# OpenVQE/OpenVQE

Hardware: AMD Instinct MI355X
Metric: vqe_energy_evals_per_sec (higher is better)
Workload: dtype f64; 1 GPU; H2O/STO-3G UCCSD energy evaluation (the metric's config): 14 qubits, 140 generators = 1000 Pauli rotations, JW Hamiltonian 1086 terms / 162 x-groups; batch_per_gpu=65536, parallelism=batch-replicas x1

## Files before the change

### openvqe_amd/csrc/abi_eval.inc

```

int ovqe_set_hamiltonian(ovqe_handle h, int64_t T, const uint64_t *x, const uint64_t *z, const double *coeff,
                         double constant) try {
    OVQE_ENTER(h);
    if (!h || T < 0 || (T && (!x || !z || !coeff))) return OVQE_ERR_INVALID;
    int rc = install_hamdev(h, h->ham, T, x, z, coeff, constant);
    if (rc) return rc;
    free_sector(h->scr);
    h->scr_failed_version = -1;
    h->user_x.assign(x, x + T);
    h->user_z.assign(z, z + T);
    h->user_c.assign(coeff, coeff + T);
    h->user_const = constant;
    h->exp_lbits = -1;
    h->sp_tried = false;
    return install_conjugated_hamiltonian(h);
} OVQE_CATCH(h)

struct FrameHamGuard {
    ovqe_handle h;
    bool on;
    explicit FrameHamGuard(ovqe_handle hh) : h(hh), on(hh && hh->frame_open && hh->ham_conj.set) {
        if (on) std::swap(h->ham, h->ham_conj);
    }
    ~FrameHamGuard() {
// ... 202 lines not shown
            }
            use_cc = C.valid;
        }
        if (use_cc && real && h->opt_sector && h->sec.valid && !h->sec.h_tables && h->sec.K == h->cc.K) {
            double2 res;
            bool ok = false;
            rc = run_sector_state(h, theta + b * (int64_t)K, (double *)h->cc.d_psic.p, &ok);
            if (rc) return rc;
            if (ok) {
                rc = run_expectation_compact(h, h->ham_real, &res, &ok, true);
                if (rc) return rc;
            }
            if (ok) {
                energies[b] = res.x + h->ham.constant;
                continue;
            }
            sector_orphaned(h);
        }
        lap("before the dense run");
        rc = run_program_streaming(h, theta + b * (int64_t)K, real);
        if (rc) return rc;
        lap("dense run");
        double2 res;
        bool tiled = false;
        if (use_cc) {
            rc = run_expectation_compact(h, h->ham_real, &res, &tiled);
            if (rc) return rc;
            if (!tiled) {
                h->cc.valid = false;
                h->cc.disabled = true;
            }
        }
        if (!tiled) rc = run_expectation_tiled(h, real ? h->ham_real : h->ham, &res, &tiled, real);
        if (rc) return rc;
        if (real && !tiled) return fail(h, OVQE_ERR_INVALID, "internal: real-amplitude path without a tile cover");
        if (!tiled)
            rc = run_bilinear(h, h->state, h->state, h->ham.groups, (const HGroup *)h->ham.d_groups.p,
                              (const HTerm *)h->ham.d_terms.p, &res, true);
        if (rc) return rc;
        lap("dense <H>");
        energies[b] = res.x + h->ham.constant;
    }
    if (!timed) {
        h->last_batch_ms = 0.f;
        return OVQE_OK;
    }
    HIPC(h, hipEventRecord(h->ev1, h->stream));
    HIPC(h, hipStreamSynchronize(h->stream));
    HIPC(h, hipEventElapsedTime(&h->last_batch_ms, h->ev0, h->ev1));
    return OVQE_OK;
} OVQE_CATCH(h)

int ovqe_energy_batch_device(ovqe_handle h, int64_t B, const void *theta_dev, int32_t K, void *energies_dev) try {
    OVQE_ENTER(h);
    if (!h || B < 0 || (B && (!theta_dev || !energies_dev))) return OVQE_ERR_INVALID;
    FrameHamGuard frame_guard(h);
    if (!h->prog_set) return fail(h, OVQE_ERR_STATE, "no program set (ovqe_set_program / ovqe_set_gate_program)");
    if (K != h->K || K <= 0) return fail(h, OVQE_ERR_INVALID, "K does not match the program's parameter count");
    if (!h->ham.set) return fail(h, OVQE_ERR_STATE, "no Hamiltonian set (ovqe_set_hamiltonian)");
    if (B == 0) return OVQE_OK;
    int rc;
    if (h->opt_force_path == 0 || h->opt_force_path == 3) {
        if (!h->sp_tried) {
            rc = build_sparse_program(h);
            if (rc) return rc;
        }
        if (h->sp_valid) {
            bool done = false;
            rc = run_sparse(h, B, (const double *)theta_dev, (double *)energies_dev, true, &done);
            if (rc || done) return rc;
        } else {
            h->sp_forms |= SPF_DECLINED;
        }
        if (h->opt_force_path == 3) return fail(h, OVQE_ERR_STATE, "program has no compact form (sparse path forced)");
    }
    if (h->n_global == 0 && h->n_local <= 16 && h->opt_force_path != 2)
        return run_small(h, B, (const double *)theta_dev, (double *)energies_dev, true);
    if (h->opt_sector_batch && h->opt_real_stream && h->prog_real_ok && h->n_global == 0 && tile_ok(h, true) && h->ham.groups.size() >= 3) {
        rc = sector_prepare(h, true);
        if (rc) return rc;
        if (sector_batch_ready(h)) {
            bool ok = false;
            rc = run_sector_energy_batch(h, B, (const double *)theta_dev, true, (double *)energies_dev, &ok);
            if (rc) return rc;
            if (ok) return OVQE_OK;
        }
    }
    std::vector<double> th((size_t)B * K), en((size_t)B);
    HIPC(h, hipMemcpyAsync(th.data(), theta_dev, th.size() * sizeof(double), hipMemcpyDeviceToHost, h->stream));
    HIPC(h, hipStreamSynchronize(h->stream));
    rc = ovqe_energy_batch(h, B, th.data(), K, en.data());
    if (rc) return rc;
    HIPC(h, hipMemcpyAsync(energies_dev, en.data(), en.size() * sizeof(double), hipMemcpyHostToDevice, h->stream));
    HIPC(h, hipStreamSynchronize(h->stream));
    return OVQE_OK;
} OVQE_CATCH(h)

int ovqe_energy(ovqe_handle h, const double *theta, int32_t K, double *energy) try {
    OVQE_ENTER(h);
    return ovqe_energy_batch(h, 1, theta, K, energy);
} OVQE_CATCH(h)

static int list_support(ovqe_handle h, uint64_t *support, bool *listed, uint64_t capacity) {
    *support = 0;
    *listed = false;
    if (h->opt_screen_sparse <= 0 || h->n_global != 0 || h->namps < 4096) return OVQE_OK;
    const uint64_t per_block = 256ull * NZ_PER_THREAD;
    const unsigned nbk = (unsigned)((h->namps + per_block - 1) / per_block);
    int rc = ensure(h, h->d_nz_cnt, (size_t)nbk * sizeof(uint32_t));
    if (!rc) rc = ensure(h, h->d_nz_start, (size_t)nbk * sizeof(uint64_t));
    if (rc) return rc;
    hipLaunchKernelGGL(k_nz_count, dim3(nbk), dim3(256), 0, h->stream, (const amp_t *)h->state, h->namps, (uint32_t *)h->d_nz_cnt.p);
    std::vector<uint32_t> cnt(nbk);
    hipError_t e = hipMemcpyAsync(cnt.data(), h->d_nz_cnt.p, (size_t)nbk * sizeof(uint32_t), hipMemcpyDeviceToHost, h->stream);
    if (e == hipSuccess) e = hipStreamSynchronize(h->stream);
    if (e != hipSuccess) return fail(h, OVQE_ERR_HIP, std::string("support list: ") + hipGetErrorString(e));
    std::vector<uint64_t> start(nbk);
    uint64_t total = 0;
    for (unsigned b = 0; b < nbk; ++b) {
        start[b] = total;
        total += cnt[b];
    }
    *support = total;
    if (total == 0 || total * (uint64_t)h->opt_screen_sparse > h->namps) return OVQE_OK;
    rc = upload(h, h->d_nz_start, start.data(), (size_t)nbk * sizeof(uint64_t));
    if (!rc) rc = ensure(h, h->d_nz_idx, std::max(total, capacity) * sizeof(uint64_t));
    if (!rc) rc = ensure(h, h->d_nz_val, total * sizeof(amp_t));
    if (rc) return rc;
    hipLaunchKernelGGL(k_nz_fill, dim3(nbk), dim3(256), 0, h->stream, (const amp_t *)h->state, h->namps,
                       (const uint64_t *)h->d_nz_start.p, (uint64_t *)h->d_nz_idx.p, (amp_t *)h->d_nz_val.p);
// ... 139 lines not shown
```

### openvqe_amd/csrc/gates_host.inc

```

void push_gate(ovqe_handle h, int opcode, int b0, int b1) {
    SmallOp op = {};
    if (opcode == OVQE_GATE_CNOT) {
        op.x = 1ull << b1;
        op.kind = OP_CNOT;
        op.first = b0;
        op.count = b1;
        op.pivot = b1;
    } else {
        op.x = 1ull << b0;
        op.kind = opcode == OVQE_GATE_X ? OP_X : OP_H;
        op.pivot = b0;
    }
    h->ops.push_back(op);
}

void push_literal_gate(ovqe_handle h, int opcode, int b0, int b1, double ascale, double aconst, int32_t pidx) {
    const uint64_t bit = 1ull << b0;
    switch (opcode) {
    case OVQE_GATE_RX: push_rotation(h, bit, 0, 0.5 * ascale, 0.5 * aconst, pidx); break;
    case OVQE_GATE_RY: push_rotation(h, bit, bit, 0.5 * ascale, 0.5 * aconst, pidx); break;
    case OVQE_GATE_RZ: push_rotation(h, 0, bit, 0.5 * ascale, 0.5 * aconst, pidx); break;
    default: push_gate(h, opcode, b0, b1);
    }
// ... 357 lines not shown
        if (poll) poll_arm(h->h_io + (size_t)B * h->K, B);
        h->cur_theta = h->d_io;
        h->cur_energies = h->d_io + (size_t)B * h->K;
    } else if (!on_device) {
        rc = ensure(h, h->d_theta, (size_t)B * std::max(1, h->K) * sizeof(double));
        if (rc) return rc;
        rc = ensure(h, h->d_energies, (size_t)B * sizeof(double));
        if (rc) return rc;
        if (h->K > 0)
            HIPC(h, hipMemcpyAsync(h->d_theta.p, theta, (size_t)B * h->K * sizeof(double), hipMemcpyHostToDevice,
                                   h->stream));
        h->cur_theta = (const double *)h->d_theta.p;
        h->cur_energies = (double *)h->d_energies.p;
    }
    SmallArgs A;
    A.n = n;
    A.K = h->K;
    A.nsegs = (int)h->segs.size();
    A.ngroups = h->exp_ngroups;
    A.nchunks = h->exp_nchunks;
    A.nflat = h->exp_nflat;
    A.cs_capacity = h->cs_capacity;
    A.B = B;
    A.constant = h->ham.constant;
    A.hf = h->hf;
    const size_t smem = small_lds(real, lds_state, n, h->cs_capacity).bytes;
    if (!zero_copy) HIPC(h, hipEventRecord(h->ev0, h->stream));
    if (real) {
        if (!lds_state) rc = launch_small<true, false, 1024, 10>(h, A, grid, smem);
        else if (nt == 1024) rc = launch_small<true, true, 1024, 10>(h, A, grid, smem);
        else if (nt == 256) rc = launch_small<true, true, 256, 8>(h, A, grid, smem);
        else rc = launch_small<true, true, 64, 6>(h, A, grid, smem);
    } else {
        if (!lds_state) rc = launch_small<false, false, 1024, 10>(h, A, grid, smem);
        else if (nt == 1024) rc = launch_small<false, true, 1024, 10>(h, A, grid, smem);
        else if (nt == 256) rc = launch_small<false, true, 256, 8>(h, A, grid, smem);
        else rc = launch_small<false, true, 64, 6>(h, A, grid, smem);
    }
    if (rc) return rc;
    h->fused_launch[0] = (real ? 1 : 0) | (lds_state ? 2 : 0) | ((nt == 1024 ? 2 : (nt == 256 ? 1 : 0)) << 2) | (zero_copy ? 16 : 0) |
                         (poll ? 32 : 0) | (on_device ? 64 : 0);
    h->fused_launch[1] = grid;
    h->fused_launch[2] = A.nsegs;
    h->fused_launch[3] = A.nchunks;
    h->fused_launch[4] = A.ngroups;
    h->fused_launch[5] = A.nflat;
    if (zero_copy) {
        if (!poll || !poll_mapped_slots(h->h_io + (size_t)B * h->K, B)) HIPC(h, hipStreamSynchronize(h->stream));
        std::memcpy(energies, h->h_io + (size_t)B * h->K, (size_t)B * sizeof(double));
        h->last_batch_ms = 0.f;
        return OVQE_OK;
    }
    HIPC(h, hipEventRecord(h->ev1, h->stream));
    if (!on_device)
        HIPC(h, hipMemcpyAsync(energies, h->cur_energies, (size_t)B * sizeof(double), hipMemcpyDeviceToHost, h->stream));
    HIPC(h, hipStreamSynchronize(h->stream));
    HIPC(h, hipEventElapsedTime(&h->last_batch_ms, h->ev0, h->ev1));
    return OVQE_OK;
}
```

### openvqe_amd/csrc/ovqe_sv.hip

```cpp
#include "../../include/ovqe_sv.h"

#include <hip/hip_runtime.h>

#include <algorithm>
#include <type_traits>
#include <atomic>
#include <cmath>
#include <cstdio>
#include <complex>
#include <cstring>
#include <map>
#include <memory>
#include <numeric>
#include <string>
#include <thread>
#include <chrono>
#include <vector>

#include "sv_kernels.hpp"
#include "sv_small.hpp"
#include "sv_sparse.hpp"
#include "sparse_pack.hpp"
#include "sv_tile.hpp"
#include "sv_sector.hpp"
// ... 332 lines not shown
    int opt_sparse_renumber = 1;
    int opt_sparse_rows = 1;
    int opt_sparse_wg = 1;
    int opt_sparse_shared = 1;
    int opt_sparse_grad = 1;
    DevBuf d_egroups, d_eterms, d_echunks, d_eflat;
    int exp_lbits = -1, exp_real = -1, exp_ngroups = 0, exp_nchunks = 0, exp_nflat = 0;
    int exp_ham_version = -1;
    hipEvent_t ev0 = nullptr, ev1 = nullptr;
    hipStream_t stream2 = nullptr;
    hipEvent_t ev_fork = nullptr, ev_join = nullptr;
    int opt_real_state = 0;
    CompactCover cc;
    int opt_compact = 1;
    int prog_version = 0;
    SectorEngine sec;
    SectorEngine scr;
    int scr_failed_version = -1;
    bool probe_independent = false;
    int opt_sector = 1;
    int opt_sector_bits = 0;
    int opt_sector_max_gb = 128;
    int opt_sector_threads = 0;
    int opt_sector_min_qubits = 18;
    int opt_sector_h = 1;
    int opt_sector_h_bits = 0;
    int opt_sector_dict = 1;
    int opt_lanczos_keep_gb = 160;
    int opt_sector_tile_cap = 6500;
    int opt_sector_sparsity = 4;
    int opt_sector_profile = 0;
    int opt_sector_debug = 0;
    int opt_sector_stream_arrange = 1;
    int opt_sector_stream_waves = 0;
    int opt_sector_sweep = 3;
    int opt_sector_sweep_dbg = 0;
    int opt_sector_h_pack = 1;
    int opt_sector_h_dbg = 0;
    int opt_sector_adjoint = 3;
    int opt_screen_sector = 1;
    int opt_screen_sector_min = 1024;
    bool prog_from_gates = false;
    int opt_expect_dense = 1;
    DevBuf d_tile_cnt;
    int opt_tile_flat = 2;
    int opt_sector_eager_rots = 2048;
    int opt_sector_regular = 1;
    int opt_sector_reg_threads = 256;
    int opt_sector_reg_adjoint = 1;
    int opt_sector_reg_pairs = 1;
    int opt_sector_reg_runs = 1;
    int opt_sector_batch = 1;
    float last_batch_ms = 0.f;
    const double *cur_theta = nullptr;
    double *cur_energies = nullptr;
    int opt_force_path = 0;
    int opt_small_max = 14;
    int opt_small_batch_max = 16;
    int opt_index_streams = 1;
    int opt_table_fusion = 1;
    int64_t last_passes = 0;
    int64_t last_pass_bytes = 0;
    int64_t last_fci_rounds = 0;
    int fault_inject = 0;
    int opt_real_mode = 1;
    int opt_tile_bits = -1;
    double2 init_amp = make_double2(1.0, 0.0);
    int opt_clifford_frame = 1;
    int opt_tile_low = 4;
    TilePlan tp;
    TilePlan tp_real;
    bool tp_real_built = false;
    bool prog_real_ok = false;
    int opt_apply_min_tiles = 256;
    int opt_real_stream = 1;
    HamDev ham_real;
    TilePlan tp_adhoc;
    TilePlan tp_adjoint;
    int opt_adjoint_tile_bits = -1;
    int num_cus = 0;
    std::vector<CrossSum *> xsums;
    std::vector<PoolPlan *> xpools;
    RdmDev *rdm = nullptr;
    int opt_rdm_workspace_mb = 1024;
    MetricDev *metric = nullptr;
    int opt_metric_workspace_mb = 0;
    MeasureDev *measure = nullptr;
    SubspaceDev *subspace = nullptr;
    int opt_subspace_workspace_mb = 0;
    HessianDev *hessian = nullptr;
};

namespace {

int rebuild_small_program(ovqe_handle h);
int build_tile_program(ovqe_handle h);
bool mapped_io(ovqe_handle h, int64_t B);

int fail(ovqe_handle h, int code, const std::string &msg) {
    if (h) h->err = msg; else g_create_error = msg;
    return code;
}

int translate_exception(ovqe_handle h) noexcept {
    int code = OVQE_ERR_INVALID;
    try {
        try {
            throw;
        } catch (const std::bad_alloc &) {
            code = OVQE_ERR_ALLOC;
            fail(h, code, "host allocation failed (std::bad_alloc)");
        } catch (const std::exception &e) {
            fail(h, code, std::string("C++ exception stopped at the ABI: ") + e.what());
        } catch (...) {
            fail(h, code, "unknown C++ exception stopped at the ABI");
        }
    } catch (...) {
    }
    return code;
}
#define OVQE_CATCH(h) catch (...) { return translate_exception(h); }

#define OVQE_ENTER(h)                        \
    do {                                     \
        if (h) {                             \
            (void)hipSetDevice((h)->device); \
            (h)->nz_super_prev = (h)->nz_super; \
            (h)->nz_super = false;           \
        }                                    \
    } while (0)

#define HIPC(h, call)                                                                                   \
    do {                                                                                                \
        hipError_t e_ = (call);                                                                         \
        if (e_ != hipSuccess)                                                                           \
            return fail(h, OVQE_ERR_HIP, std::string(#call) + ": " + hipGetErrorString(e_));            \
    } while (0)

constexpr size_t LDS_WG_MAX = 160 * 1024;
constexpr size_t LDS_WG_BUDGET = 150 * 1024;
constexpr size_t LDS_TWO_PER_CU = 80 * 1024;
constexpr size_t SEC_LDS_MAX = 156 * 1024;

template <auto Kernel>
int lds_opt_in(ovqe_handle h, size_t bytes) {
    static std::atomic<bool> done[64];
    std::atomic<bool> &d = done[h->device & 63];
    if (!d.load(std::memory_order_acquire)) {
        HIPC(h, hipFuncSetAttribute(reinterpret_cast<const void *>(Kernel), hipFuncAttributeMaxDynamicSharedMemorySize, (int)bytes));
        d.store(true, std::memory_order_release);
    }
    return OVQE_OK;
}
template <auto K0, auto K1, auto... Ks>
int lds_opt_in(ovqe_handle h, size_t bytes) {
    const int rc = lds_opt_in<K0>(h, bytes);
    return rc ? rc : lds_opt_in<K1, Ks...>(h, bytes);
}

void free_hamdev(HamDev &H) {
    for (DevBuf *b : {&H.d_groups, &H.d_terms, &H.d_tchunks, &H.d_tgroups, &H.d_tterms, &H.d_tflats, &H.d_titems, &H.d_rest, &H.d_achunks,
                      &H.d_agroups, &H.d_aterms, &H.d_dzin, &H.d_doff, &H.d_dterms})
        if (b->p) {
            (void)hipFree(b->p);
            *b = DevBuf{};
        }
}

void free_cross_sum(CrossSum *X) {
    if (!X) return;
    free_hamdev(X->local);
    for (DevBuf *b : {&X->local_cover.d_achunks, &X->local_cover.d_agroups, &X->local_cover.d_aterms, &X->local_cover.d_groups, &X->local_cover.d_terms})
        if (b->p) (void)hipFree(b->p);
    for (int f = 0; f < 2; ++f)
        for (CrossCoverDev &C : X->partners[f])
            for (DevBuf *b : {&C.d_achunks, &C.d_agroups, &C.d_aterms, &C.d_groups, &C.d_terms})
                if (b->p) (void)hipFree(b->p);
    if (X->d_part.p) (void)hipFree(X->d_part.p);
    delete X;
}

void free_pool_plan(PoolPlan *P) {
    if (!P) return;
    for (int f = 0; f < 2; ++f)
        for (PoolCoverDev &D : P->covers[f])
            for (DevBuf *b : {&D.d_chunks, &D.d_entries, &D.d_terms})
                if (b->p) (void)hipFree(b->p);
    for (DevBuf *b : {&P->d_part, &P->d_out})
        if (b->p) (void)hipFree(b->p);
    delete P;
}

void release_block(void *p, size_t cap) {
    if (!p) return;
    if (DevBlockCache::current && DevBlockCache::current->blocks.size() < 512) DevBlockCache::current->blocks.push_back(DevBuf{p, cap});
    else (void)hipFree(p);
}

constexpr uint64_t OVQE_POLL_SENTINEL = 0x7ff8dead0badf00dull;
inline bool poll_mapped_slot(volatile uint64_t *slot) {
    const auto t0 = std::chrono::steady_clock::now();
    for (uint32_t spins = 0; *slot == OVQE_POLL_SENTINEL; ++spins) {
        __builtin_ia32_pause();
        if ((spins & 1023u) == 1023u && std::chrono::steady_clock::now() - t0 > std::chrono::milliseconds(5)) return false;
    }
    std::atomic_thread_fence(std::memory_order_acquire);
    return true;
}

inline void poll_arm(double *slots, int64_t B) {
    for (int64_t b = 0; b < B; ++b) std::memcpy(slots + b, &OVQE_POLL_SENTINEL, sizeof(uint64_t));
}
inline bool poll_mapped_slots(double *slots, int64_t B) {
    for (int64_t b = 0; b < B; ++b)
        if (!poll_mapped_slot(reinterpret_cast<volatile uint64_t *>(slots + b))) return false;
    return true;
}

int ensure(ovqe_handle h, DevBuf &b, size_t bytes) {
    if (b.cap >= bytes && b.p) return OVQE_OK;
    release_block(b.p, b.cap);
    b.p = nullptr;
    b.cap = 0;
    size_t want = std::max<size_t>(bytes, 256);
    if (DevBlockCache::current) {
        if (want < ((size_t)8 << 20)) {
            size_t base = 256;
            while (base * 2 <= want) base *= 2;
            const size_t step = base / 4;
            want = base + ((want - base + step - 1) / step) * step;
        }
        size_t cap = 0;
        if (void *p = DevBlockCache::current->take(want, &cap)) {
            b.p = p;
            b.cap = cap;
            return OVQE_OK;
        }
    }
    hipError_t e = hipMalloc(&b.p, want);
    if (e != hipSuccess && DevBlockCache::current && !DevBlockCache::current->blocks.empty()) {
        (void)hipGetLastError();
        DevBlockCache::current->flush();
        e = hipMalloc(&b.p, want);
    }
    if (e != hipSuccess) return fail(h, OVQE_ERR_ALLOC, std::string("hipMalloc: ") + hipGetErrorString(e));
    b.cap = want;
    return OVQE_OK;
}

int ensure_scratch(ovqe_handle h, int k) {
    if (h->scratch[k]) return OVQE_OK;
    hipError_t e = hipMalloc((void **)&h->scratch[k], h->namps * sizeof(amp_t));
    if (e != hipSuccess) return fail(h, OVQE_ERR_ALLOC, std::string("hipMalloc scratch: ") + hipGetErrorString(e));
    return OVQE_OK;
}

inline uint64_t local_mask(ovqe_handle h) { return h->namps - 1ull; }
inline int reduce_blocks(uint64_t namps) {
    return (int)std::min<uint64_t>(2048, std::max<uint64_t>(1, (namps + 255) / 256));
}

inline int enqueue_reduce(ovqe_handle h, const void *partials, int64_t count, int slot = 0) {
    hipLaunchKernelGGL(k_reduce, dim3(1), dim3(256), 0, h->stream, (const double2 *)partials, count, (double2 *)h->d_result.p, slot);
    HIPC(h, hipGetLastError());
    return OVQE_OK;
}
inline int fetch_result(ovqe_handle h, double2 *out, int nslots = 1) {
    HIPC(h, hipMemcpyAsync(h->h_result, h->d_result.p, (size_t)nslots * sizeof(double2), hipMemcpyDeviceToHost, h->stream));
    HIPC(h, hipStreamSynchronize(h->stream));
    std::copy(h->h_result, h->h_result + nslots, out);
    return OVQE_OK;
}
inline int reduce_to_host(ovqe_handle h, const void *partials, int64_t count, double2 *out) {
// ... 1 lines not shown
    return fetch_result(h, out);
}
inline int reduce_to_host(ovqe_handle h, const void *partials, int64_t count, double *re) {
    double2 sum = make_double2(0.0, 0.0);
    const int rc = reduce_to_host(h, partials, count, &sum);
    *re = sum.x;
    return rc;
}

int build_groups(ovqe_handle h, int64_t T, const uint64_t *x, const uint64_t *z, const double *cr, const double *ci,
                 bool allow_global_x, std::vector<HGroup> &groups, std::vector<HTerm> &terms,
                 std::vector<uint64_t> *xs_out = nullptr, std::vector<int64_t> *perm_out = nullptr) {
    const uint64_t lmask = local_mask(h);
    const int ntot = h->n_local + h->n_global;
    const uint64_t allmask = ntot >= 64 ? ~0ull : ((1ull << ntot) - 1ull);
    if (h->fault_inject == 1) {
        h->fault_inject = 0;
        throw std::bad_alloc();
    }
    std::vector<int64_t> order(T);
    std::iota(order.begin(), order.end(), 0);
    std::stable_sort(order.begin(), order.end(), [&](int64_t a, int64_t b) { return x[a] < x[b]; });
    groups.clear();
    terms.clear();
    terms.reserve(T);
    for (int64_t oi = 0; oi < T; ++oi) {
        const int64_t t = order[oi];
        if ((x[t] | z[t]) & ~allmask) return fail(h, OVQE_ERR_INVALID, "Pauli mask has bits beyond the register");
        if (!allow_global_x && (x[t] & ~lmask))
            return fail(h, OVQE_ERR_INVALID,
                        "x mask touches global (rank) bits: exchange shards first (openvqe_amd/distributed.py)");
        HTerm ht;
        ht.z = z[t];
        fold_iny(cr[t], ci ? ci[t] : 0.0, __builtin_popcountll(x[t] & z[t]), ht.cr, ht.ci);
        if (groups.empty() || x[order[oi - 1]] != x[t]) {
            HGroup g;
            g.x = x[t] & lmask;
            g.jbase = (h->base ^ x[t]) & ~lmask;
            g.t0 = (int32_t)terms.size();
            g.t1 = g.t0;
            g.tiny = 0.0;
            groups.push_back(g);
        }
        terms.push_back(ht);
        groups.back().t1 = (int32_t)terms.size();
        groups.back().tiny += 64.0 * 2.220446049250313e-16 * (std::fabs(ht.cr) + std::fabs(ht.ci));
        if (xs_out) xs_out->push_back(x[t] & lmask);
    }
    if (perm_out) *perm_out = order;
    return OVQE_OK;
}

int upload(ovqe_handle h, DevBuf &b, const void *src, size_t bytes) {
    int rc = ensure(h, b, bytes);
    if (rc) return rc;
    if (bytes) HIPC(h, hipMemcpyAsync(b.p, src, bytes, hipMemcpyHostToDevice, h->stream));
    HIPC(h, hipStreamSynchronize(h->stream));
    return OVQE_OK;
}

int launch_rot_run(ovqe_handle h, uint64_t x, const RotParam *d_rp, int nrot) {
    if (nrot <= 0) return OVQE_OK;
    const int nl = h->n_local;
    if (x == 0) {
        const uint64_t n = h->namps;
#define OVQE_LAUNCH_D(NT, U, NTL)                                                                                \
    hipLaunchKernelGGL((k_rot_diag_v<NT, U, NTL>), dim3((unsigned)((n + (uint64_t)NT * U - 1) / ((uint64_t)NT * U))), \
                       dim3(NT), 0, h->stream, h->state, n, h->base, d_rp, nrot);
        if (nl >= 32) {
            OVQE_LAUNCH_D(64, 4, true)
        } else if (nl >= 21 && nl < 25) {
            OVQE_LAUNCH_D(256, 1, false)
        } else if (nl >= 14) {
            OVQE_LAUNCH_D(64, 1, true)
        } else if (n >= 256u * 4u) {
            hipLaunchKernelGGL(k_rot_diag<4>, dim3((unsigned)((n + 1023) / 1024)), dim3(256), 0, h->stream, h->state,
                               n, h->base, d_rp, nrot);
        } else {
            hipLaunchKernelGGL(k_rot_diag<1>, dim3((unsigned)((n + 255) / 256)), dim3(256), 0, h->stream, h->state,
                               n, h->base, d_rp, nrot);
        }
#undef OVQE_LAUNCH_D
    } else {
        const uint64_t np = h->namps >> 1;
        const int pivot = 63 - __builtin_clzll(x);
#define OVQE_LAUNCH_V(NT, U, NTL)                                                                                    \
    hipLaunchKernelGGL((k_rot_pairs_v<NT, U, NTL>), dim3((unsigned)((np + (uint64_t)NT * U - 1) / ((uint64_t)NT * U))), \
                       dim3(NT), 0, h->stream, h->state, np, pivot, x, h->base, d_rp, nrot);
        if (nl >= 32) {
            OVQE_LAUNCH_V(64, 4, true)
        } else if (nl >= 25 && pivot < 7) {
            OVQE_LAUNCH_V(128, 1, true)
        } else if (nl >= 21 && nl < 25) {
            OVQE_LAUNCH_V(256, 1, false)
        } else if (nl >= 14) {
            OVQE_LAUNCH_V(64, 1, true)
        } else if (np >= 256u * 4u) {
            hipLaunchKernelGGL(k_rot_pairs<4>, dim3((unsigned)((np + 1023) / 1024)), dim3(256), 0, h->stream,
                               h->state, np, pivot, x, h->base, d_rp, nrot);
        } else if (np >= 256u * 2u) {
            hipLaunchKernelGGL(k_rot_pairs<2>, dim3((unsigned)((np + 511) / 512)), dim3(256), 0, h->stream, h->state,
                               np, pivot, x, h->base, d_rp, nrot);
        } else {
            hipLaunchKernelGGL(k_rot_pairs<1>, dim3((unsigned)((np + 255) / 256)), dim3(256), 0, h->stream, h->state,
                               np, pivot, x, h->base, d_rp, nrot);
        }
#undef OVQE_LAUNCH_V
// ... 335 lines not shown
    h->shard = shard;
    h->namps = 1ull << n_local;
    h->base = shard << n_local;
    if (adopt) {
        h->state = (amp_t *)adopt;
        h->own_state = false;
    } else {
        e = hipMalloc((void **)&h->state, h->namps * sizeof(amp_t));
        if (e != hipSuccess) {
            delete h;
            return fail(nullptr, OVQE_ERR_ALLOC, std::string("hipMalloc state: ") + hipGetErrorString(e));
        }
    }
    if (hipHostMalloc((void **)&h->h_result, 64 * sizeof(double2), hipHostMallocDefault) != hipSuccess ||
        hipEventCreate(&h->ev0) != hipSuccess || hipEventCreate(&h->ev1) != hipSuccess) {
        if (h->own_state) (void)hipFree(h->state);
        delete h;
        return fail(nullptr, OVQE_ERR_ALLOC, "host staging / event creation failed");
    }
    *out = h;
    return OVQE_OK;
}

}

extern "C" {

int ovqe_version(void) { return 100; }

const char *ovqe_last_error(ovqe_handle h) { return h ? h->err.c_str() : g_create_error.c_str(); }

int ovqe_device_count(int *count) {
    if (!count) return OVQE_ERR_INVALID;
    int c = 0;
    if (hipGetDeviceCount(&c) != hipSuccess) c = 0;
    *count = c;
    return OVQE_OK;
}

int ovqe_create(int n_qubits, int device, ovqe_handle *out) try {
    return create_common(n_qubits, 0, 0, device, out);
} OVQE_CATCH(nullptr)

int ovqe_create_shard(int n_local, int n_global, uint64_t shard_index, int device, ovqe_handle *out) try {
    return create_common(n_local, n_global, shard_index, device, out);
} OVQE_CATCH(nullptr)

int ovqe_create_view(int n_qubits, int device, void *dev_ptr, ovqe_handle *out) try {
    if (!dev_ptr) return fail(nullptr, OVQE_ERR_INVALID, "dev_ptr is NULL");
    return create_common(n_qubits, 0, 0, device, out, dev_ptr);
} OVQE_CATCH(nullptr)

int ovqe_destroy(ovqe_handle h) try {
    OVQE_ENTER(h);
    if (!h) return OVQE_OK;
    (void)hipSetDevice(h->device);
    (void)hipStreamSynchronize(h->stream);
    if (h->own_state && h->state) (void)hipFree(h->state);
    for (int k = 0; k < 2; ++k)
        if (h->scratch[k]) (void)hipFree(h->scratch[k]);
    std::vector<DevBuf *> bufs = {&h->d_tile_cnt, &h->d_partials, &h->d_result, &h->d_rp, &h->d_ops, &h->d_rots, &h->d_rots_seq, &h->d_segs,
                                  &h->d_stream,
                                  &h->d_theta, &h->d_energies, &h->d_workspace, &h->d_egroups, &h->d_eterms, &h->d_echunks,
                                  &h->d_eflat, &h->d_sp_ops, &h->d_sp_rows, &h->d_sp_rows64, &h->d_sp_prim, &h->d_sp_pairs, &h->d_sp_entries, &h->d_sp_hpack, &h->d_pg_off, &h->d_pg_xs, &h->d_pg_terms, &h->d_pg_runs, &h->d_pg_tabs,
                                  &h->d_pg_out, &h->d_pg_part, &h->d_nz_cnt, &h->d_nz_start, &h->d_nz_idx, &h->d_nz_val, &h->d_nz_bitmap, &h->d_exp_groups, &h->d_exp_terms, &h->d_tile_smasks, &h->d_tile_lists, &h->d_tile_counts, &h->cc.d_sup, &h->cc.d_psic, &h->cc.d_loc, &h->cc.d_cid, &h->cc.d_off, &h->cc.d_sweeps};
    for (TilePlan *tp : {&h->tp, &h->tp_adhoc, &h->tp_real, &h->tp_adjoint}) bufs.insert(bufs.end(), {&tp->d_tops, &tp->d_trots});
    for (HamDev *H : {&h->ham, &h->ham_adhoc, &h->ham_real, &h->ham_conj})
        bufs.insert(bufs.end(), {&H->d_groups, &H->d_terms, &H->d_tchunks, &H->d_tgroups, &H->d_tterms, &H->d_tflats,
                                 &H->d_titems, &H->d_rest, &H->d_achunks, &H->d_agroups, &H->d_aterms, &H->d_dzin, &H->d_doff, &H->d_dterms});
    for (DevBuf *b : bufs)
        if (b->p) (void)hipFree(b->p);
    free_sector(h->sec);
    free_sector(h->scr);
    for (CrossSum *X : h->xsums) free_cross_sum(X);
    for (PoolPlan *P : h->xpools) free_pool_plan(P);
    free_rdm(h->rdm);
    free_metric(h->metric);
    free_measure(h->measure);
    free_subspace(h->subspace);
    free_hessian(h->hessian);
    h->kept_blocks.flush();
    if (h->h_rp) (void)hipHostFree(h->h_rp);
    if (h->h_result) (void)hipHostFree(h->h_result);
    if (h->h_io) (void)hipHostFree(h->h_io);
    if (h->h_fin) (void)hipHostFree(h->h_fin);
    if (h->ev0) (void)hipEventDestroy(h->ev0);
    if (h->ev1) (void)hipEventDestroy(h->ev1);
    if (h->ev_fork) (void)hipEventDestroy(h->ev_fork);
    if (h->ev_join) (void)hipEventDestroy(h->ev_join);
    if (h->stream2) (void)hipStreamDestroy(h->stream2);
    delete h;
    return OVQE_OK;
} OVQE_CATCH(h)

int ovqe_set_stream(ovqe_handle h, void *hip_stream) try {
    OVQE_ENTER(h);
    if (!h) return OVQE_ERR_INVALID;
    HIPC(h, hipStreamSynchronize(h->stream));
    h->stream = (hipStream_t)hip_stream;
    return OVQE_OK;
} OVQE_CATCH(h)

static void reset_sector(ovqe_handle h) {
    free_sector(h->sec);
    h->sec.disabled = false;
    h->sec.seen = 0;
    h->sec.prog_version = -1;
}
// ... 248 lines not shown
    const int nb = reduce_blocks(h->namps);
    int rc = ensure(h, h->d_partials, (size_t)nb * sizeof(double2));
    if (!rc) rc = ensure(h, h->d_result, 64 * sizeof(double2));
    if (rc) return rc;
    hipLaunchKernelGGL(k_norm2, dim3(nb), dim3(256), 0, h->stream, h->state, h->opt_real_state ? std::max<uint64_t>(h->namps >> 1, 1) : h->namps,
                       (double2 *)h->d_partials.p);
    return reduce_to_host(h, h->d_partials.p, nb, out);
} OVQE_CATCH(h)

#include "abi_unit.inc"

#include "abi_eval.inc"

#include "abi_adapt.inc"

#include "abi_solvers.inc"

#include "abi_rdm.inc"

#include "abi_metric.inc"

#include "abi_measure.inc"

#include "abi_subspace.inc"

#include "abi_hessian.inc"

int ovqe_time_pauli_rotation(ovqe_handle h, uint64_t x, uint64_t z, double phi, int warmup, int reps, double *avg_ms) try {
    OVQE_ENTER(h);
    if (!h || !avg_ms || reps <= 0 || warmup < 0) return OVQE_ERR_INVALID;
    if (x & ~local_mask(h)) return fail(h, OVQE_ERR_INVALID, "x mask touches global (rank) bits");
    int rc = ensure_rp(h, 1);
    if (rc) return rc;
    h->h_rp[0] = make_rot(x, z, phi);
    HIPC(h, hipMemcpyAsync(h->d_rp.p, h->h_rp, sizeof(RotParam), hipMemcpyHostToDevice, h->stream));
    for (int i = 0; i < warmup; ++i) {
        rc = launch_rot_run(h, x, (const RotParam *)h->d_rp.p, 1);
        if (rc) return rc;
    }
    HIPC(h, hipEventRecord(h->ev0, h->stream));
    for (int i = 0; i < reps; ++i) {
        rc = launch_rot_run(h, x, (const RotParam *)h->d_rp.p, 1);
        if (rc) return rc;
    }
    HIPC(h, hipEventRecord(h->ev1, h->stream));
    HIPC(h, hipStreamSynchronize(h->stream));
    float ms = 0.f;
    HIPC(h, hipEventElapsedTime(&ms, h->ev0, h->ev1));
    *avg_ms = (double)ms / reps;
    return OVQE_OK;
} OVQE_CATCH(h)

int ovqe_program_info(ovqe_handle h, int64_t *info, int count) try {
    OVQE_ENTER(h);
    if (!h || !info || count < 0) return OVQE_ERR_INVALID;
    if (!h->prog_set) return fail(h, OVQE_ERR_STATE, "no program set");
    const bool real_on = h->opt_real_stream && h->prog_real_ok && h->n_global == 0 && tile_ok(h, true);
    const HamDev &HI = (real_on && h->ham_real.version == h->ham.version) ? h->ham_real : h->ham;
    const TilePlan &TP = (real_on && h->tp_real_built) ? h->tp_real : h->tp;
    int64_t v[16] = {(int64_t)h->ops.size(), (int64_t)h->rots.size(), 0, (int64_t)TP.plan.size(),
                     (int64_t)TP.tsegs.size(), (int64_t)h->sops.size(),
                     !h->sp_tried ? -1 : (h->sp_valid ? (int64_t)h->sp_m : 0),
                     (int64_t)HI.tsweeps.size(), (int64_t)HI.n_rest, HI.tile_entries, HI.tile_terms, HI.tile_work,
                     real_on ? 1 : 0, h->sp_valid ? (int64_t)h->sp_nops : 0, h->sp_valid ? (int64_t)h->sp_npairs : 0,
                     h->sp_valid ? (int64_t)h->sp_nent : 0};
    for (const SmallOp &op : h->ops) v[2] += (op.kind == OP_X || op.kind == OP_H || op.kind == OP_CNOT);
    for (int i = 0; i < count && i < 16; ++i) info[i] = v[i];
    const SectorEngine &E = h->sec;
    const int64_t sv[14] = {E.valid ? (int64_t)E.K : 0, E.valid ? (int64_t)E.segs.size() : 0, E.valid ? (int64_t)E.npairs : 0,
                           E.valid ? (int64_t)E.hs.size() : 0, E.valid ? (int64_t)E.nnz : 0, E.valid ? (int64_t)E.bytes : 0,
                           E.valid ? (int64_t)(1e3 * E.last_circuit_ms) : 0, E.valid ? (int64_t)(1e3 * E.last_expect_ms) : 0,
                           E.valid ? (int64_t)E.h_stream_bytes : 0, E.valid ? (int64_t)E.last_fci_block : 0,
                            h->sp_valid ? h->sp_conflicts_before : 0, h->sp_valid ? h->sp_conflicts_after : 0,
                            (E.valid && E.regular && h->opt_sector_regular) ? (int64_t)E.reg_m : 0,
                            (E.valid && E.regular) ? (int64_t)__builtin_popcount(E.freemask) : 0};
    for (int i = 16; i < count && i < 30; ++i) info[i] = sv[i - 16];
    const bool packed = h->sp_valid && h->sp_pack_inst >= 0;
    const int64_t pv[3] = {packed ? (int64_t)h->sp_h_pieces : 0, packed ? (int64_t)h->sp_h_rpt * h->sp_h_epr : 0,
                           packed ? (int64_t)h->sp_h_rpt * (h->sp_h_epr + 1) : 0};
    for (int i = 30; i < count && i < 33; ++i) info[i] = pv[i - 30];
    for (int i = 33; i < count && i < 38; ++i) info[i] = h->sp_valid ? h->sp_cycles[i - 33] : 0;
    int64_t dict_entries = 0, ordered = 0;
    for (const SectorHSweep &hw : E.hs) dict_entries += hw.ndict;
    for (const SectorSeg &sg : E.segs) ordered += sg.d_torder.p ? 1 : 0;
    const int64_t gv[8] = {E.valid ? (int64_t)E.M : 0, E.valid ? (int64_t)E.Mh : 0, E.valid ? (int64_t)E.sb : 0, E.valid ? (int64_t)E.max_tile : 0,
                           E.valid ? (int64_t)E.h_max_tile : 0, E.valid ? (int64_t)E.h_max_dict : 0, E.valid ? dict_entries : 0,
                           E.valid ? ordered : 0};
    for (int i = 38; i < count && i < 46; ++i) info[i] = gv[i - 38];
    return OVQE_OK;
} OVQE_CATCH(h)

int ovqe_get_rotation_program(ovqe_handle h, int64_t capacity, uint64_t *x, uint64_t *z, double *coeff, double *phi0,
                              int32_t *pidx, int64_t *count) try {
    OVQE_ENTER(h);
    if (!h || !count || capacity < 0 || (capacity > 0 && (!x || !z || !coeff || !phi0 || !pidx))) return OVQE_ERR_INVALID;
    if (!h->prog_set) return fail(h, OVQE_ERR_STATE, "no program set");
    if (h->frame_open) return fail(h, OVQE_ERR_STATE, "the program's Clifford frame is open: the rotations alone are not the circuit");
    int64_t n = 0;
    for (const SmallOp &op : h->ops) {
        if (op.kind != OP_PAIR && op.kind != OP_DIAG) return fail(h, OVQE_ERR_STATE, "the program holds literal X / H / CNOT ops");
        for (int32_t r = op.first; r < op.first + op.count; ++r, ++n) {
            if (n >= capacity) continue;
            const SmallRot &sr = h->rots[r];
            x[n] = op.x;
            z[n] = sr.z;
            coeff[n] = sr.coeff;
            phi0[n] = sr.phi0;
            pidx[n] = sr.pidx;
        }
    }
    *count = n;
    return OVQE_OK;
} OVQE_CATCH(h)

int ovqe_last_support(ovqe_handle h, int32_t which, int64_t *support) try {
    OVQE_ENTER(h);
    if (!h || !support || which < 0 || which > 13) return OVQE_ERR_INVALID;
    const int64_t v[8] = {h->last_screen_support, h->last_exp_support, h->last_screen_sector, h->last_fci_rounds, h->last_passes, h->last_pass_bytes,
                          (int64_t)h->forms_used, (int64_t)h->sp_forms};
    *support = which < 8 ? v[which] : h->fused_launch[which - 8];
    return OVQE_OK;
} OVQE_CATCH(h)

int ovqe_last_batch_ms(ovqe_handle h, double *ms) try {
    OVQE_ENTER(h);
    if (!h || !ms) return OVQE_ERR_INVALID;
    *ms = h->last_batch_ms;
    return OVQE_OK;
} OVQE_CATCH(h)

}

#include "cross_host.inc"
#include "pool_host.inc"
```

### openvqe_amd/csrc/sparse_host.inc

```

struct SharedInstance { int nw, ept, sstride, rpt, epr, te; };
constexpr SharedInstance SHARED_13 = {4, 13, 2568, 1, 17, 3};
constexpr SharedInstance SHARED_37 = {4, 37, 4104, 4, 10, 5};
constexpr SharedInstance SHARED_INSTANCES[2] = {SHARED_13, SHARED_37};

int build_sparse_program(ovqe_handle h) {
    h->sp_tried = true;
    h->sp_valid = false;
    if (!h->opt_sparse || !h->opt_table_fusion || !h->opt_real_mode || h->n_global != 0 || h->n_local > 40) return OVQE_OK;
    if (!h->prog_set || !h->ham.set || h->K <= 0) return OVQE_OK;
    for (const SmallRot &sr : h->rots)
        if (!(sr.ny & 1)) return OVQE_OK;
    for (const SmallOp &op : h->sops)
        if (op.kind != OP_TAB || op.count > 127) return OVQE_OK;
    const int MAXM = 4096;
    std::unordered_map<uint64_t, int> id;
    std::vector<uint64_t> S;
    auto get = [&](uint64_t a) {
        auto it = id.find(a);
        if (it != id.end()) return it->second;
        const int k = (int)S.size();
        id.emplace(a, k);
        S.push_back(a);
        return k;
// ... 369 lines not shown
        bool shared = false;
        if ((B >= SHARED_MIN_B && h->opt_sparse_shared) || h->opt_sparse_shared >= 2) {
            if (!rc && !shared) {
                rc = launch_rows_shared<0>(h, R, &shared);
                if (shared) h->sp_forms |= SPG_SHARED_13;
            }
            if (!rc && !shared) {
                rc = launch_rows_shared<1>(h, R, &shared);
                if (shared) h->sp_forms |= SPG_SHARED_37;
            }
            if (rc) return rc;
        }
        if (!shared) {
#define OVQE_ROWS(DBG_)                                                                                                                       \
    do {                                                                                                                                      \
        rc = lds_opt_in<&k_sparse_vqe_rows<2, DBG_>>(h, LDS_WG_MAX);                                                                          \
        if (rc) return rc;                                                                                                                    \
        hipLaunchKernelGGL((k_sparse_vqe_rows<2, DBG_>), dim3(grid), dim3(64), sp_rows_lds(R, 2).bytes, h->stream, R, h->cur_theta,            \
                           (const SmallRot *)h->d_sp_prim.p, (const uint64_t *)h->d_sp_rows.p, h->sp_nrows4, (const SpEntry *)h->d_sp_entries.p, \
                           h->cur_energies);                                                                                                  \
    } while (0)
            switch (h->opt_sparse_dbg) {
            case 1: OVQE_ROWS(1); break;
            case 2: OVQE_ROWS(2); break;
            case 3: OVQE_ROWS(3); break;
#ifdef OVQE_TESTING
            case 5: OVQE_ROWS(5); break;
#endif
            default: OVQE_ROWS(0);
            }
#undef OVQE_ROWS
            HIPC(h, hipGetLastError());
            h->sp_forms |= SPG_PER_WAVE;
        }
        h->sp_forms |= SPF_ROWS2;
    }
    else if (spw == 2) {
        rc = launch_sparse<2>(h, A, grid, sp_vqe_lds(A, 2, false).bytes);
        h->sp_forms |= SPF_PLAIN2;
    }
    else {
        rc = launch_sparse<1>(h, A, grid, sp_vqe_lds(A, 1, false).bytes);
        h->sp_forms |= SPF_PLAIN1;
    }
    if (rc) return rc;
    *done = true;
    if (zero_copy) {
        if (!poll || !poll_mapped_slots(h->h_io + (size_t)B * h->K, B)) HIPC(h, hipStreamSynchronize(h->stream));
        std::memcpy(energies, h->h_io + (size_t)B * h->K, (size_t)B * sizeof(double));
        h->last_batch_ms = 0.f;
        return OVQE_OK;
    }
    HIPC(h, hipEventRecord(h->ev1, h->stream));
    if (!on_device)
        HIPC(h, hipMemcpyAsync(energies, h->cur_energies, (size_t)B * sizeof(double), hipMemcpyDeviceToHost, h->stream));
    HIPC(h, hipStreamSynchronize(h->stream));
    HIPC(h, hipEventElapsedTime(&h->last_batch_ms, h->ev0, h->ev1));
    return OVQE_OK;
}

int run_sparse_gradient(ovqe_handle h, const double *theta, double *energy, double *grad, bool *done) {
    *done = false;
    if (!(h->opt_force_path == 0 || h->opt_force_path == 3) || !h->opt_sparse_grad || h->n_local > 16) return OVQE_OK;
    int rc = OVQE_OK;
    if (!h->sp_tried) {
        rc = build_sparse_program(h);
        if (rc) return rc;
    }
    if (!h->sp_valid) {
        h->sp_forms |= SPF_DECLINED;
        return OVQE_OK;
    }
    SparseArgs A;
    A.m = h->sp_mp;
    A.mpad = (h->sp_mp + 1) & ~1;
    A.hf = h->sp_hf;
    A.K = h->K;
    A.nops = h->sp_nops;
    A.ntab = (int)h->srots.size();
    A.nent = h->sp_nent;
    A.npairs = (int)h->sp_npairs;
    A.B = 1;
    A.constant = h->ham.constant;
    const size_t base = sp_grad_lds(A, false).bytes, staged = sp_grad_lds(A, true).bytes;
    if (base > LDS_WG_BUDGET) {
        h->sp_forms |= SPF_DECLINED;
        return OVQE_OK;
    }
    const bool stage = staged <= LDS_WG_BUDGET;
    rc = lds_opt_in<&k_sparse_grad<true>, &k_sparse_grad<false>>(h, LDS_WG_MAX);
    if (rc) return rc;
    const bool zero_copy = mapped_io(h, 2);
    const double *d_theta;
    double *d_e, *d_g;
    if (zero_copy) {
        std::memcpy(h->h_io, theta, (size_t)h->K * sizeof(double));
        d_theta = h->d_io;
        d_e = h->d_io + h->K;
        d_g = h->d_io + h->K + 1;
    } else {
        rc = ensure(h, h->d_theta, (size_t)std::max(1, h->K) * sizeof(double));
        if (!rc) rc = ensure(h, h->d_energies, (size_t)(h->K + 1) * sizeof(double));
        if (rc) return rc;
        HIPC(h, hipMemcpyAsync(h->d_theta.p, theta, (size_t)h->K * sizeof(double), hipMemcpyHostToDevice, h->stream));
        d_theta = (const double *)h->d_theta.p;
        d_e = (double *)h->d_energies.p;
        d_g = d_e + 1;
    }
// ... 38 lines not shown
```

Baseline: 184.4 million evals/s.

## Return device-resident batch energy calls without stream sync, drain lazily

```diff
diff --git a/openvqe_amd/csrc/abi_eval.inc b/openvqe_amd/csrc/abi_eval.inc
--- a/openvqe_amd/csrc/abi_eval.inc
+++ b/openvqe_amd/csrc/abi_eval.inc
@@ -278,7 +278,7 @@
 } OVQE_CATCH(h)
 
 int ovqe_energy_batch_device(ovqe_handle h, int64_t B, const void *theta_dev, int32_t K, void *energies_dev) try {
-    OVQE_ENTER(h);
+    OVQE_ENTER_ASYNC(h);
     if (!h || B < 0 || (B && (!theta_dev || !energies_dev))) return OVQE_ERR_INVALID;
     FrameHamGuard frame_guard(h);
     if (!h->prog_set) return fail(h, OVQE_ERR_STATE, "no program set (ovqe_set_program / ovqe_set_gate_program)");
@@ -288,6 +288,7 @@
     int rc;
     if (h->opt_force_path == 0 || h->opt_force_path == 3) {
         if (!h->sp_tried) {
+            if (h->batch_pending) return fail(h, OVQE_ERR_STATE, "internal: compact tables to build under a batch in flight");
             rc = build_sparse_program(h);
             if (rc) return rc;
         }
@@ -302,6 +303,7 @@
     }
     if (h->n_global == 0 && h->n_local <= 16 && h->opt_force_path != 2)
         return run_small(h, B, (const double *)theta_dev, (double *)energies_dev, true);
+    if ((rc = drain_pending(h))) return rc;
     if (h->opt_sector_batch && h->opt_real_stream && h->prog_real_ok && h->n_global == 0 && tile_ok(h, true) && h->ham.groups.size() >= 3) {
         rc = sector_prepare(h, true);
         if (rc) return rc;
diff --git a/openvqe_amd/csrc/gates_host.inc b/openvqe_amd/csrc/gates_host.inc
--- a/openvqe_amd/csrc/gates_host.inc
+++ b/openvqe_amd/csrc/gates_host.inc
@@ -433,8 +433,11 @@
         return OVQE_OK;
     }
     HIPC(h, hipEventRecord(h->ev1, h->stream));
-    if (!on_device)
-        HIPC(h, hipMemcpyAsync(energies, h->cur_energies, (size_t)B * sizeof(double), hipMemcpyDeviceToHost, h->stream));
+    if (on_device) {
+        h->batch_pending = true;
+        return OVQE_OK;
+    }
+    HIPC(h, hipMemcpyAsync(energies, h->cur_energies, (size_t)B * sizeof(double), hipMemcpyDeviceToHost, h->stream));
     HIPC(h, hipStreamSynchronize(h->stream));
     HIPC(h, hipEventElapsedTime(&h->last_batch_ms, h->ev0, h->ev1));
     return OVQE_OK;
diff --git a/openvqe_amd/csrc/ovqe_sv.hip b/openvqe_amd/csrc/ovqe_sv.hip
--- a/openvqe_amd/csrc/ovqe_sv.hip
+++ b/openvqe_amd/csrc/ovqe_sv.hip
@@ -408,6 +408,7 @@
     int opt_sector_reg_runs = 1;
     int opt_sector_batch = 1;
     float last_batch_ms = 0.f;
+    bool batch_pending = false;
     const double *cur_theta = nullptr;
     double *cur_energies = nullptr;
     int opt_force_path = 0;
@@ -477,7 +478,7 @@
 }
 #define OVQE_CATCH(h) catch (...) { return translate_exception(h); }
 
-#define OVQE_ENTER(h)                        \
+#define OVQE_ENTER_ASYNC(h)                  \
     do {                                     \
         if (h) {                             \
             (void)hipSetDevice((h)->device); \
@@ -485,6 +486,12 @@
             (h)->nz_super = false;           \
         }                                    \
     } while (0)
+#define OVQE_ENTER(h)                                 \
+    do {                                              \
+        OVQE_ENTER_ASYNC(h);                          \
+        if ((h) && (h)->batch_pending)                \
+            if (int rc_ = drain_pending(h)) return rc_; \
+    } while (0)
 
 #define HIPC(h, call)                                                                                   \
     do {                                                                                                \
@@ -492,6 +499,15 @@
         if (e_ != hipSuccess)                                                                           \
             return fail(h, OVQE_ERR_HIP, std::string(#call) + ": " + hipGetErrorString(e_));            \
     } while (0)
+
+int drain_pending(ovqe_handle h) {
+    if (!h->batch_pending) return OVQE_OK;
+    h->batch_pending = false;
+    h->last_batch_ms = 0.f;
+    HIPC(h, hipEventSynchronize(h->ev1));
+    HIPC(h, hipEventElapsedTime(&h->last_batch_ms, h->ev0, h->ev1));
+    return OVQE_OK;
+}
 
 constexpr size_t LDS_WG_MAX = 160 * 1024;
 constexpr size_t LDS_WG_BUDGET = 150 * 1024;
@@ -575,6 +591,8 @@
 
 int ensure(ovqe_handle h, DevBuf &b, size_t bytes) {
     if (b.cap >= bytes && b.p) return OVQE_OK;
+    if (h && h->batch_pending)
+        if (int rc = drain_pending(h)) return rc;
     release_block(b.p, b.cap);
     b.p = nullptr;
     b.cap = 0;
@@ -682,7 +700,8 @@
 }
 
 int upload(ovqe_handle h, DevBuf &b, const void *src, size_t bytes) {
-    int rc = ensure(h, b, bytes);
+    int rc = h->batch_pending ? drain_pending(h) : OVQE_OK;
+    if (!rc) rc = ensure(h, b, bytes);
     if (rc) return rc;
     if (bytes) HIPC(h, hipMemcpyAsync(b.p, src, bytes, hipMemcpyHostToDevice, h->stream));
     HIPC(h, hipStreamSynchronize(h->stream));
@@ -1124,8 +1143,9 @@
 } OVQE_CATCH(nullptr)
 
 int ovqe_destroy(ovqe_handle h) try {
-    OVQE_ENTER(h);
+    OVQE_ENTER_ASYNC(h);
     if (!h) return OVQE_OK;
+    (void)drain_pending(h);
     (void)hipSetDevice(h->device);
     (void)hipStreamSynchronize(h->stream);
     if (h->own_state && h->state) (void)hipFree(h->state);
@@ -1480,7 +1500,7 @@
 } OVQE_CATCH(h)
 
 int ovqe_program_info(ovqe_handle h, int64_t *info, int count) try {
-    OVQE_ENTER(h);
+    OVQE_ENTER_ASYNC(h);
     if (!h || !info || count < 0) return OVQE_ERR_INVALID;
     if (!h->prog_set) return fail(h, OVQE_ERR_STATE, "no program set");
     const bool real_on = h->opt_real_stream && h->prog_real_ok && h->n_global == 0 && tile_ok(h, true);
@@ -1542,7 +1562,7 @@
 } OVQE_CATCH(h)
 
 int ovqe_last_support(ovqe_handle h, int32_t which, int64_t *support) try {
-    OVQE_ENTER(h);
+    OVQE_ENTER_ASYNC(h);
     if (!h || !support || which < 0 || which > 13) return OVQE_ERR_INVALID;
     const int64_t v[8] = {h->last_screen_support, h->last_exp_support, h->last_screen_sector, h->last_fci_rounds, h->last_passes, h->last_pass_bytes,
                           (int64_t)h->forms_used, (int64_t)h->sp_forms};
@@ -1551,8 +1571,9 @@
 } OVQE_CATCH(h)
 
 int ovqe_last_batch_ms(ovqe_handle h, double *ms) try {
-    OVQE_ENTER(h);
+    OVQE_ENTER_ASYNC(h);
     if (!h || !ms) return OVQE_ERR_INVALID;
+    if (int rc = drain_pending(h)) return rc;
     *ms = h->last_batch_ms;
     return OVQE_OK;
 } OVQE_CATCH(h)
diff --git a/openvqe_amd/csrc/sparse_host.inc b/openvqe_amd/csrc/sparse_host.inc
--- a/openvqe_amd/csrc/sparse_host.inc
+++ b/openvqe_amd/csrc/sparse_host.inc
@@ -445,8 +445,11 @@
         return OVQE_OK;
     }
     HIPC(h, hipEventRecord(h->ev1, h->stream));
-    if (!on_device)
-        HIPC(h, hipMemcpyAsync(energies, h->cur_energies, (size_t)B * sizeof(double), hipMemcpyDeviceToHost, h->stream));
+    if (on_device) {
+        h->batch_pending = true;
+        return OVQE_OK;
+    }
+    HIPC(h, hipMemcpyAsync(energies, h->cur_energies, (size_t)B * sizeof(double), hipMemcpyDeviceToHost, h->stream));
     HIPC(h, hipStreamSynchronize(h->stream));
     HIPC(h, hipEventElapsedTime(&h->last_batch_ms, h->ev0, h->ev1));
     return OVQE_OK;
```

Result: no change. 184.2 million evals/s (-0.2%).
